# open-rmf/rmf_crowdsim

Hardware: AMD Instinct MI355X
Metric: agent-steps/sec at 1M agents, dt=0.05 s; % HBM roofline on Zanlungo kernel (higher is better)
Workload: dtype f32

## Files before the change

### include/crowdstep.h

```cpp
#ifndef CROWDSTEP_H
#define CROWDSTEP_H

#include <stddef.h>
#include <stdint.h>

#ifdef __cplusplus
extern "C" {
#endif

#define CS_ABI_VERSION 1

typedef struct cs_engine cs_engine;

typedef struct cs_grid_desc {
  double width;
  double height;
  double cell_size;
  double offset_x;
  double offset_y;
} cs_grid_desc;

typedef struct cs_device_cfg {
  int32_t device_ordinal;
  uint32_t flags;
// ... 112 lines not shown

uint32_t cs_abi_version(void);
cs_engine* cs_create(const cs_grid_desc* grid, const cs_device_cfg* cfg);
void cs_destroy(cs_engine*);
const char* cs_last_error(const cs_engine*);
const char* cs_backend_name(const cs_engine*);

uint32_t cs_register_zanlungo(cs_engine*, const cs_zanlungo_params*);
uint32_t cs_register_no_local_plan(cs_engine*);
uint32_t cs_register_lp_callback(cs_engine*, cs_lp_batch_fn fn, void* user);
uint32_t cs_register_hlp(cs_engine*, const cs_hlp_desc*);

int cs_add_agents(cs_engine*, const double* xy, size_t n, uint32_t hlp,
                  uint32_t lp, double eyesight, uint64_t* out_ids);
int cs_remove_agent(cs_engine*, uint64_t id);
uint32_t cs_add_source_sink(cs_engine*, const cs_source_sink_desc*);
void cs_remove_source_sink(cs_engine*, uint32_t handle);
size_t cs_source_sink_slots(cs_engine*);

int cs_step(cs_engine*, double dt_seconds, cs_step_report* report);
int cs_synchronize(cs_engine*);

size_t cs_agent_count(cs_engine*);
size_t cs_read_agents(cs_engine*, cs_agent_view* out, size_t cap);
size_t cs_drain_events(cs_engine*, cs_event* out, size_t cap);
void cs_event_recording(cs_engine*, int on);
typedef struct cs_snapshot_record {
  double x, y;
  float vx, vy;
  uint32_t id;
  uint32_t next_waypoint;
} cs_snapshot_record;
int cs_snapshot_request(cs_engine*);
int cs_snapshot_acquire(cs_engine*, int wait, const cs_snapshot_record** out,
                        size_t* n, uint64_t* step_index);
size_t cs_query_radius(cs_engine*, double radius, double x, double y,
                       uint64_t* out_ids, size_t cap);
size_t cs_query_knn(cs_engine*, size_t k, double x, double y, uint64_t* out_ids);

int cs_query_radius_batch(cs_engine*, size_t n, const double* xy, const double* radius, size_t cap_per_query,
                          uint64_t* out_ids, uint64_t* out_counts, float* out_d2, uint32_t* out_cells);
int cs_query_knn_batch(cs_engine*, size_t n, const double* xy, size_t k, uint64_t* out_ids, uint64_t* out_counts,
                       float* out_d2);

uint64_t cs_device_bytes(cs_engine*);

#define CS_STAT_WINDOWS_OFF_LDS 0u
#define CS_STAT_WINDOWS_CHUNKED 1u
#define CS_STAT_EXCHANGES_AHEAD 2u
#define CS_STAT_EXCHANGES_AHEAD_USED 3u
#define CS_STAT_STEPS_ON_KEPT_WINDOWS 4u
#define CS_STAT_RENUMBERINGS 5u
#define CS_STAT_RENUMBER_NS 6u
uint64_t cs_kernel_stat(cs_engine*, uint32_t which);

enum {
  CS_K_NEIGHBOUR_FORCE = 0,
  CS_K_SCAN = 1,
  CS_K_SCATTER = 2,
  CS_K_SPAWN = 3,
  CS_K_HALO = 4,
  CS_K_HALO_PACK = 5,
  CS_K_HALO_EXCHANGE = 6,
  CS_K_HALO_UNPACK = 7,
  CS_K_STEP_BORDER = 8,
  CS_K_STEP_INTERIOR = 9,
  CS_K_COUNT = 10
};
void cs_profile_enable(cs_engine*, uint32_t kernel_mask);
void cs_profile_stride(cs_engine*, uint32_t every);
int cs_profile_read(cs_engine*, uint32_t kernel, double* total_ms, uint64_t* launches);
void cs_profile_reset(cs_engine*);

enum { CS_DIR_XLO = 0, CS_DIR_XHI = 1, CS_DIR_YLO = 2, CS_DIR_YHI = 3,
       CS_DIR_XLO_YLO = 4, CS_DIR_XLO_YHI = 5, CS_DIR_XHI_YLO = 6, CS_DIR_XHI_YHI = 7 };
#define CS_HALO_RECORD_BYTES 40u
int cs_halo_set_buffers(cs_engine*, uint32_t dir, void* send_dev, void* recv_dev,
                        uint64_t capacity_records);
int cs_halo_pack(cs_engine*, uint32_t axis);
int cs_halo_unpack(cs_engine*, uint32_t axis);
int cs_halo_pack_all(cs_engine*);
int cs_halo_unpack_all(cs_engine*);
size_t cs_spawn_probe(cs_engine*, double dt_seconds, uint8_t* flags, size_t cap);
int cs_spawn_commit(cs_engine*, const uint8_t* flags, size_t n);
int cs_spawn_probe_dev(cs_engine*, double dt_seconds, int* flags_dev, size_t cap);
int cs_spawn_commit_dev(cs_engine*, const int* flags_dev, size_t n);

int cs_tile_histogram(cs_engine*, uint64_t* rows, uint64_t* cols);
size_t cs_tile_export(cs_engine*, void* records, size_t cap_records);
int cs_tile_retile(cs_engine*, uint32_t tile_cx0, uint32_t tile_cx1, uint32_t tile_cy0, uint32_t tile_cy1);
int cs_tile_import(cs_engine*, const void* records, size_t n);

typedef struct cs_route_miss {
  uint64_t id;
  uint32_t hlp;
  uint32_t slot;
  double px, py;
  double tx, ty;
} cs_route_miss;
size_t cs_route_misses(cs_engine*, cs_route_miss* out, size_t cap);
int cs_route_resolve(cs_engine*, const cs_route_miss* all, size_t n);

#define CS_RCCL_UNIQUE_ID_BYTES 128
int cs_rccl_unique_id(uint8_t* out_id);
int cs_rccl_comm_init(cs_engine*, int32_t n_ranks, int32_t rank, const uint8_t* id);
int cs_rccl_comm_adopt(cs_engine*, void* nccl_comm);
// ... 64 lines not shown
```

### rmf_crowdsim_amd/_abi.py

```python
import ctypes as C

CS_ABI_VERSION = 1

CS_CFG_DEFAULT = 0
CS_CFG_FORCE_GATHER = 1
CS_CFG_FORCE_TILED = 2
CS_CFG_DENSE = 4
CS_CFG_TILE_OVERLAP = 8
CS_CFG_WIDE_IDS = 16
CS_STAT_WINDOWS_OFF_LDS = 0
CS_STAT_WINDOWS_CHUNKED = 1
CS_STAT_EXCHANGES_AHEAD = 2
CS_STAT_EXCHANGES_AHEAD_USED = 3
CS_STAT_STEPS_ON_KEPT_WINDOWS = 4
CS_STAT_RENUMBERINGS = 5
CS_STAT_RENUMBER_NS = 6

CS_HLP_NONE, CS_HLP_CONSTANT, CS_HLP_ID_PARITY, CS_HLP_CALLBACK, CS_HLP_ROUTE = 0, 1, 2, 3, 4
CS_ROUTE_MAX_WAYPOINTS = 1023
CS_GEN_MONOTONIC, CS_GEN_POISSON_SEEDED, CS_GEN_CALLBACK = 0, 1, 2
CS_EVENT_SPAWNED, CS_EVENT_DESTROYED = 1, 2
(CS_K_NEIGHBOUR_FORCE, CS_K_SCAN, CS_K_SCATTER, CS_K_SPAWN, CS_K_HALO, CS_K_HALO_PACK, CS_K_HALO_EXCHANGE,
 CS_K_HALO_UNPACK, CS_K_STEP_BORDER, CS_K_STEP_INTERIOR, CS_K_COUNT) = range(11)
KERNEL_NAMES = ["neighbour_force", "scan", "scatter", "spawn", "halo", "halo_pack", "halo_exchange", "halo_unpack",
                "step_border", "step_interior"]
CS_DIR_XLO, CS_DIR_XHI, CS_DIR_YLO, CS_DIR_YHI = 0, 1, 2, 3
CS_DIR_XLO_YLO, CS_DIR_XLO_YHI, CS_DIR_XHI_YLO, CS_DIR_XHI_YHI = 4, 5, 6, 7
CS_HALO_RECORD_BYTES = 40
CS_RCCL_UNIQUE_ID_BYTES = 128
NO_SOURCE_SINK = 0xFFFFFFFF


class GridDesc(C.Structure):
    _fields_ = [("width", C.c_double), ("height", C.c_double), ("cell_size", C.c_double),
                ("offset_x", C.c_double), ("offset_y", C.c_double)]


class DeviceCfg(C.Structure):
    _fields_ = [("device_ordinal", C.c_int32), ("flags", C.c_uint32),
                ("tile_cx0", C.c_uint32), ("tile_cx1", C.c_uint32),
                ("tile_cy0", C.c_uint32), ("tile_cy1", C.c_uint32),
                ("halo_cells", C.c_uint32), ("reserved", C.c_uint32),
                ("capacity_hint", C.c_uint64), ("stream", C.c_void_p)]


class ZanlungoParams(C.Structure):
    _fields_ = [("agent_scale", C.c_double), ("obstacle_scale", C.c_double),
                ("reaction_time", C.c_double), ("force_distance", C.c_double),
                ("agent_mass", C.c_double), ("agent_radius", C.c_double)]


HlpVelocityFn = C.CFUNCTYPE(None, C.c_void_p, C.c_size_t, C.POINTER(C.c_uint64),
                            C.POINTER(C.c_double), C.POINTER(C.c_double), C.c_double,
                            C.POINTER(C.c_double), C.POINTER(C.c_uint8))
HlpSetTargetFn = C.CFUNCTYPE(None, C.c_void_p, C.c_uint64, C.c_double, C.c_double, C.c_double,
                             C.c_double, C.c_double, C.c_double)
HlpRemoveFn = C.CFUNCTYPE(None, C.c_void_p, C.c_uint64)
GeneratorFn = C.CFUNCTYPE(C.c_size_t, C.c_void_p, C.c_double)


class LpAgent(C.Structure):
    _fields_ = [("agent_id", C.c_uint64), ("x", C.c_double), ("y", C.c_double), ("vx", C.c_double),
                ("vy", C.c_double), ("preferred_vx", C.c_double), ("preferred_vy", C.c_double),
                ("eyesight_range", C.c_double), ("next_waypoint", C.c_uint64)]


LpBatchFn = C.CFUNCTYPE(C.c_int, C.c_void_p, C.c_size_t, C.POINTER(LpAgent), C.POINTER(C.c_double),
                        C.POINTER(C.c_uint64), C.POINTER(LpAgent), C.POINTER(C.c_double))

# ... 242 lines not shown
```

### rmf_crowdsim_amd/csrc/crowdstep_hip.hip

```cpp

#include <hip/hip_runtime.h>
#include <chrono>

#include <algorithm>
#include <cmath>
#include <cstdint>
#include <cstdio>
#include <array>
#include <cmath>
#include <cstring>
#include <map>
#include <string>
#include <thread>
#include <tuple>
#include <vector>

#include "crowdstep.h"
#include "crowdstep_state.h"

#define CS_INVALID_CELL 0xFFFFFFFFu
#define CS_MAX_GROUPS 1048575u
#define CS_SPAWN_OCCUPANCY_RADIUS 0.4
#define CS_ID_LIMIT 0x7FFFFFFFull

// ... 246 lines not shown
      ev.x = ev.y = 0;
      if (e->record_events) e->events.push_back(ev);
      return 0;
    }
  if (int rc = e->refresh_counts()) return rc;
  uint32_t found[2] = {0xFFFFFFFFu, 0u};
  uint64_t dev = 0;
  if (e->dev_id(id, &dev) && dev < 0xFFFFFFFFull && e->n_slots) {
    if (!e->find_dev && hipMalloc(&e->find_dev, 2 * sizeof(uint32_t)) != hipSuccess) {
      e->error = "HIP error while removing an agent";
      return 90;
    }
    bool ok = hipMemcpyAsync(e->find_dev, found, sizeof found, hipMemcpyHostToDevice, e->stream) == hipSuccess;
    hipLaunchKernelGGL(k_remove_by_id, dim3((e->n_slots + 255u) / 256u), dim3(256), 0, e->stream, e->buf[e->cur],
                       e->n_slots, e->ctr, e->gdev.tile, (uint32_t)dev, e->find_dev);
    ok = ok && hipMemcpyAsync(found, e->find_dev, sizeof found, hipMemcpyDeviceToHost, e->stream) == hipSuccess &&
         hipStreamSynchronize(e->stream) == hipSuccess;
    if (!ok) {
      e->error = "HIP error while removing an agent";
      return 90;
    }
  }
  if (found[0] == 0xFFFFFFFFu) {
    e->error = "unknown agent id";
    return 2;
  }
  const HostGroup& g = e->groups[meta_group(e->gdev, found[1])];
  const cs_hlp_desc& p = e->hlps[g.hlp];
  if (p.kind == CS_HLP_CALLBACK && p.remove_agent) p.remove_agent(p.user, id);
  e->sorted = false;
  e->hist_valid = false;
  e->occ_valid = false;
  e->halo_invalidate();
  e->n_alive_host -= 1;
  cs_event ev;
  ev.kind = CS_EVENT_DESTROYED;
  ev.source_sink = g.sink >= 0 ? (uint32_t)g.sink : UINT32_MAX;
  ev.id = id;
  ev.x = ev.y = 0;
  if (e->record_events) e->events.push_back(ev);
  return 0;
}

size_t cs_source_sink_slots(cs_engine* e) { return e->sinks.size(); }
uint64_t cs_device_bytes(cs_engine* e) { return e->device_bytes(); }

uint64_t cs_kernel_stat(cs_engine* e, uint32_t which) {
  hipSetDevice(e->device);
  if (which == CS_STAT_EXCHANGES_AHEAD) return e->n_exchanges_ahead;
  if (which == CS_STAT_EXCHANGES_AHEAD_USED) return e->n_exchanges_ahead_used;
  if (which == CS_STAT_STEPS_ON_KEPT_WINDOWS) return e->n_steps_on_kept_windows;
  if (which == CS_STAT_RENUMBERINGS) return e->n_renumberings;
  if (which == CS_STAT_RENUMBER_NS) return e->renumber_ns;
  Counters c;
  if (e->read_counters(&c)) return 0;
  switch (which) {
    case CS_STAT_WINDOWS_OFF_LDS: return c.n_win_off_lds;
    case CS_STAT_WINDOWS_CHUNKED: return c.n_win_chunked;
#ifdef CS_TILE_TRIPS
    case 100: case 101: case 102: case 103: case 104: case 105: case 106: case 107: case 108: case 109: case 110: case 111:
    case 112: case 113: case 114: case 115: case 116:
      return c.dbg[which - 100];
#endif
    default: return 0;
  }
}

uint32_t cs_add_source_sink(cs_engine* e, const cs_source_sink_desc* d) {
  if (d->n_waypoints == 0) {
    e->error = "a source-sink needs at least one waypoint";
    return UINT32_MAX;
  }
  hipSetDevice(e->device);
  if (e->room_for_group(d->n_waypoints)) return UINT32_MAX;
  HostSink s;
  s.d = *d;
  s.waypoints.assign(d->waypoints_xy, d->waypoints_xy + 2 * d->n_waypoints);
  s.d.waypoints_xy = nullptr;
  uint32_t handle = (uint32_t)e->sinks.size();
  if (e->tile && d->hlp < e->hlps.size() && e->hlps[d->hlp].kind == CS_HLP_ROUTE) {
    s.spawn_route = e->route_lookup(d->hlp, d->source_x, d->source_y, s.waypoints[0], s.waypoints[1]);
    if (!s.spawn_route) {
      e->error = "route planner found no route for this source-sink (tile engines plan at registration)";
      return UINT32_MAX;
    }
  }
  s.group = e->make_group(d->hlp, d->lp, d->agent_eyesight_range, (int32_t)handle);
  e->sinks.push_back(s);
  e->sinks_dirty = true;
  return handle;
}

void cs_remove_source_sink(cs_engine* e, uint32_t handle) {
  if (handle < e->sinks.size() && e->sinks[handle].alive) {
    e->sinks[handle].alive = false;
    e->sinks_dirty = true;
  }
}

int cs_step(cs_engine* e, double dt_seconds, cs_step_report* report) {
  hipSetDevice(e->device);
  const int rc = e->step(dt_seconds, report);
  if (rc == 0) e->steps_done += 1;
  return rc;
}

// ... 760 lines not shown
```

### rmf_crowdsim_amd/csrc/cs_engine.hip.inc

```

namespace {

inline uint64_t sat_usize(double v) {
  if (!(v > 0.0)) return 0;
  if (v >= 18446744073709551615.0) return UINT64_MAX;
  return (uint64_t)v;
}

inline uint64_t splitmix64(uint64_t x) {
  x += 0x9E3779B97F4A7C15ull;
  x = (x ^ (x >> 30)) * 0xBF58476D1CE4E5B9ull;
  x = (x ^ (x >> 27)) * 0x94D049BB133111EBull;
  return x ^ (x >> 31);
}
inline uint64_t poisson_seeded(uint64_t seed, uint64_t step, double mean) {
  if (!(mean > 0.0)) return 0;
  double limit = std::exp(-mean), prod = 1.0;
  uint64_t k = 0;
  for (uint64_t draw = 0; draw < 1000000; ++draw) {
    uint64_t r = splitmix64(seed ^ splitmix64(step * 0x100000001B3ull + draw));
    double u = (double)((r >> 11) + 1) * (1.0 / 9007199254740993.0);
    prod *= u;
    if (prod <= limit) break;
    ++k;
// ... 728 lines not shown
    if (hist_valid) return 0;
    HIP_OK(hipMemsetAsync(cell_count, 0, (ncells + 1) * sizeof(uint32_t), stream));
    if (n_slots)
      hipLaunchKernelGGL(k_count, dim3((n_slots + 255) / 256), dim3(256), 0, stream, buf[cur], 0u,
                         n_slots, cell_count, ctr, gdev.tile);
    HIP_OK(hipGetLastError());
    hist_valid = true;
    return 0;
  }

  uint32_t tile_agents_cap(int h) const {
    const uint32_t rb = tile_rows;
    if (rb <= 1)
      return std::min<uint32_t>(TILE_AGENTS_MAX, ((uint32_t)(2 * h + 1) * TILE_THREADS * 9u / 8u + 192u + tile_agents_slack + 63u) & ~63u);
    const double per_cell = (double)n_slots / (double)std::max<uint64_t>(ncells, 1);
    const double halo_cols = 2.0 * h * per_cell * 1.25;
    const double want = (rb + 2.0 * h) * ((double)tile_target / rb * 9.0 / 8.0 + halo_cols) + 64.0 + tile_agents_slack;
    const uint32_t base = ((rb + 2u * h) * (tile_target / rb) * 9u / 8u + 192u + tile_agents_slack + 63u) & ~63u;
    const uint32_t cap = std::max(base, ((uint32_t)want + 63u) & ~63u);
    return std::min<uint32_t>(TILE_AGENTS_MAX, cap);
  }

  bool bands_built = false;
  bool windows_shadow = true;
  uint32_t windows_keep_max_agents = 300000, windows_slack_pct = 10;
  bool windows_valid = false;
  bool scan_onepass = true;
  unsigned long long* scan_tile_sums = nullptr;
  uint32_t scan_seq = 0;
  uint32_t debug_sort_every = 0, debug_sort_phase = 0, debug_sorted_slots = 0;
  bool debug_sorted_once = false;
  bool debug_ctx_by_value = false;
  uint32_t scan_ticket_base = 0;
  uint32_t kept_agents_cap = 0;
  uint32_t windows_bound = 0;
  BlockDesc* blk_desc_back = nullptr;
  uint32_t* n_blocks_back = nullptr;
  struct WindowsKey {
    uint32_t ncells, nx, own_x0, own_x1, own_y0, own_y1, org_x, org_y, h, desc_cap, rows, target, stage_cap, split;
    const void* desc;
    bool operator==(const WindowsKey& o) const { return std::memcmp(this, &o, sizeof *this) == 0; }
  } windows_key{};
  int alloc_window_arrays(uint32_t cap_each) {
    hipFree(blk_desc);
    hipFree(blk_desc_back);
    blk_desc = blk_desc_back = nullptr;
    blk_desc_cap = cap_each;
    HIP_OK(hipMalloc(&blk_desc, (uint64_t)blk_desc_cap * sizeof(BlockDesc)));
    HIP_OK(hipMalloc(&blk_desc_back, (uint64_t)blk_desc_cap * sizeof(BlockDesc)));
    windows_valid = false;
    return 0;
  }
  uint64_t n_steps_on_kept_windows = 0;
  bool check_windows = false;
  std::string check_windows_error;
  int check_window_list(const BlockDesc* list_dev, const uint32_t* count_dev, uint32_t rows, uint32_t n_bands, uint32_t max_cols,
                        bool cover, uint32_t launch_windows) {
    HIP_OK(hipStreamSynchronize(stream));
    uint32_t cnt[2] = {0, 0};
    HIP_OK(hipMemcpy(cnt, count_dev, sizeof cnt, hipMemcpyDeviceToHost));
    char msg[512];
    if (cnt[0] > blk_desc_cap || cnt[0] > launch_windows) {
      std::snprintf(msg, sizeof msg, "window check: %u windows listed, the array holds %u, the launch %u", cnt[0], blk_desc_cap, launch_windows);
      check_windows_error = msg;
      error = check_windows_error.c_str();
      return 7;
    }
    std::vector<BlockDesc> d(cnt[0]);
    if (cnt[0]) HIP_OK(hipMemcpy(d.data(), list_dev, (size_t)cnt[0] * sizeof(BlockDesc), hipMemcpyDeviceToHost));
    const uint32_t ncols = gdev.own_y1 - gdev.own_y0;
    std::vector<std::vector<uint8_t>> seen(n_bands, std::vector<uint8_t>(cover ? ncols : 0u, 0));
    for (uint32_t k = 0; k < cnt[0]; ++k) {
      const BlockDesc& w = d[k];
      const bool in_rows = w.row0 >= gdev.own_x0 && w.row0 < gdev.own_x1 && (w.row0 - gdev.own_x0) % rows == 0u && w.nrows >= 1u &&
                           w.nrows <= rows && w.row0 + w.nrows <= gdev.own_x1;
      const bool in_cols = w.y0 <= w.y1 && w.y0 >= gdev.own_y0 && w.y1 < gdev.own_y1 &&
                           (w.y1 - w.y0 + 1u <= max_cols || ncols > BAND_LDS_COLS);
      if (!in_rows || !in_cols || w.count != 0u) {
        std::snprintf(msg, sizeof msg, "window check: window %u of %u is {row0 %u nrows %u y0 %u y1 %u first %u count %u}; owned rows [%u, %u) columns [%u, %u), %u rows per band, %u columns at most",
                      k, cnt[0], w.row0, w.nrows, w.y0, w.y1, w.first, w.count, gdev.own_x0, gdev.own_x1, gdev.own_y0, gdev.own_y1, rows, max_cols);
        check_windows_error = msg;
        error = check_windows_error.c_str();
        return 7;
      }
      if (cover) {
        std::vector<uint8_t>& band = seen[(w.row0 - gdev.own_x0) / rows];
        for (uint32_t y = w.y0; y <= w.y1; ++y) band[y - gdev.own_y0] += 1;
      }
    }
    if (cover)
      for (uint32_t b = 0; b < n_bands; ++b)
        for (uint32_t y = 0; y < ncols; ++y)
          if (seen[b][y] != 1) {
            std::snprintf(msg, sizeof msg, "window check: column %u of band %u is covered %u times (%u windows)", y, b, (unsigned)seen[b][y], cnt[0]);
            check_windows_error = msg;
            error = check_windows_error.c_str();
            return 7;
          }
    return 0;
  }
  uint32_t tile_max_cols(uint32_t h) const {
    const long long half = (long long)FIX_LIM / std::max(gdev.cs_fix, 1) - 2;
    const long long cols = 2 * half - 2 * (long long)h - 2;
    return (uint32_t)std::max<long long>(1, std::min<long long>(cols, 4096));
  }
  uint32_t split_margin() const {
    const bool wanted = ((flags & CS_CFG_TILE_OVERLAP) && rccl_comm != nullptr) || tile_split_force;
    return (tile && wanted && tile_rows > 1) ? halo_cells + 1u : 0u;
  }
  int rebuild(uint32_t bands = 0, uint32_t band_rows = 0, uint32_t band_h = 0, uint32_t band_stage_cap = 0,
              bool keep_windows = false, bool cover = false, uint32_t band_target = 0) {
    const bool bands_were_built = bands_built;
    bands_built = false;
    if (sorted) return 0;
    if (int rc = recount()) return rc;
    if (debug_sort_every > 1 && !tile && n_live_sinks == 0 && debug_sorted_once && !keep_windows && n_slots == debug_sorted_slots &&
        (++debug_sort_phase % debug_sort_every) != 0) {
      HIP_OK(hipMemsetAsync(cell_count, 0, (size_t)ncells * sizeof(uint32_t), stream));
      HIP_OK(hipMemsetAsync(&ctr->n_destroyed, 0, 6 * sizeof(uint32_t), stream));
      bands_built = bands_were_built;
      sorted = true;
      hist_valid = false;
      return 0;
    }
    debug_sorted_once = true;
    debug_sorted_slots = n_slots;
    prof_begin(CS_K_SCAN);
    uint32_t* const scan_clears = (keep_windows || windows_valid) ? n_blocks_back : n_blocks_dev;
    if (scan_onepass && n_scan_blocks <= SCAN_ONEPASS_MAX_BLOCKS) {
      if (!scan_tile_sums) {
        HIP_OK(hipMalloc(&scan_tile_sums, ((size_t)SCAN_ONEPASS_MAX_BLOCKS + 1) * sizeof(unsigned long long)));
        HIP_OK(hipMemsetAsync(scan_tile_sums, 0, ((size_t)SCAN_ONEPASS_MAX_BLOCKS + 1) * sizeof(unsigned long long), stream));
        scan_ticket_base = 0;
      }
      if (++scan_seq == 0u) scan_seq = 1u;
      hipLaunchKernelGGL(k_scan_onepass, dim3(n_scan_blocks), dim3(SCAN_BLOCK), 0, stream, cell_count, (uint32_t)ncells,
                         cell_start, ctr, scan_clears, scan_tile_sums, scan_seq,
                         reinterpret_cast<uint32_t*>(scan_tile_sums + SCAN_ONEPASS_MAX_BLOCKS), scan_ticket_base);
      scan_ticket_base += n_scan_blocks;
    } else {
// ... 1000 lines not shown
        if (++early_seq == 0u) early_seq = 1u;
        c2.flag_seq = early_seq;
        StepParams Pc = P;
        Pc.halo_late_check = fuse_pack ? 1u : 0u;
        {
          const dim3 grid(grid_blocks), block(TILE_THREADS);
          const EpilogueCore& Ec = static_cast<const EpilogueCore&>(E);
          if (ctx_by_value)
            hipLaunchKernelGGL((k_step_tiled<true, false, true>), grid, block, lds, stream, Pc, view(cur), Ep, Ec, cell_start, pref, blk_desc, n_blocks_dev, c2);
          else
            hipLaunchKernelGGL((k_step_tiled<false, false, true>), grid, block, lds, stream, Pc, view(cur), Ep, Ec, cell_start, pref, blk_desc, n_blocks_dev, c2);
        }
        border_on_aux = true;
        early_pending = true;
      } else if (n_slots && split) {
        TileCfg cfg_b = cfg;
        cfg_b.part = 1;
        cfg_b.spill = tile_spill + (uint64_t)grid_blocks * cfg.spill_rows * TILE_THREADS;
        hipStream_t sb = stream;
        border_on_aux = false;
        if (overlap_ready && (!need_host || fire_and_forget)) {
          if (int rc = ensure_aux()) return rc;
          HIP_OK(hipEventRecord(ev_sorted, stream));
          HIP_OK(hipStreamWaitEvent(aux_stream, ev_sorted, 0));
          sb = aux_stream;
          border_on_aux = true;
        }
        const int tb = prof_open_on(CS_K_STEP_BORDER, sb);
        launch_tiled(sb, P, cfg_b);
        prof_close_on(tb, sb);
        if (border_on_aux) HIP_OK(hipEventRecord(ev_border, aux_stream));
        StepParams Pi = P;
        Pi.halo_late_check = fuse_pack ? 1u : 0u;
        const int ti = prof_open_on(CS_K_STEP_INTERIOR, stream);
        launch_tiled(stream, Pi, cfg);
        prof_close_on(ti, stream);
        if (border_on_aux) HIP_OK(hipStreamWaitEvent(stream, ev_border, 0));
      } else if (n_slots) {
        launch_tiled(stream, P, cfg);
      }
      prof_end();
    } else {
      if (tile)
        hipLaunchKernelGGL(k_build_blocks, dim3(1), dim3(1024), 0, stream, gdev, cell_start, blk_desc,
                           blk_desc_cap, n_blocks_dev, ctr);
      if (n_slots && P.peek_seq) flight_launched(P.peek_seq);
      prof_begin(CS_K_NEIGHBOUR_FORCE);
      if (n_slots)
        hipLaunchKernelGGL(k_step_gather, dim3((n_slots + 255) / 256), dim3(256), 0, stream, P, view(cur),
                           Ep, cell_start, pref);
      prof_end();
    }
    HIP_OK(hipGetLastError());
    if (builders && check_windows)
      if (int rc = check_window_list(blk_desc_back, n_blocks_back, tile_rows, n_bands, tile_max_cols((uint32_t)h), true, 0xFFFFFFFFu)) return rc;
    if (builders) {
      std::swap(blk_desc, blk_desc_back);
      std::swap(n_blocks_dev, n_blocks_back);
    }
    windows_valid = want_keep && n_slots != 0u && tiled && (builders != 0u || (keep_now && had_windows) || (!keep_now && bands_built) || cover_built_late);
    if (windows_valid && (builders != 0u || !keep_now)) windows_bound = band_windows_max;
    if (windows_valid) kept_agents_cap = agents_cap_now;
    if (fuse_pack) {
      halo_prepacked = true;
      halo_all_clean = false;
      halo_counts_clean[0] = halo_counts_clean[1] = false;
    }

    if (!need_host || fire_and_forget) {
      cur ^= 1;
      sorted = false;
      hist_valid = true;
      occ_valid = has_sinks;
      if (has_sinks || tile) {
        counts_stale = true;
        ++async_steps;
      }
      errors_stale = true;
      spawn_committed = false;
      committed_spawns = 0;
      slots_added = 0;
      ghosts_present = false;
      return 0;
    }

    Counters c;
    if (int rc = read_counters(&c)) return rc;
    counts_stale = false;
    errors_stale = false;
    async_steps = 0;
    if (has_sinks && (!tile || spawn_on_device)) next_id = c.next_id;
    const uint64_t first_spawn_id = (uint64_t)c.next_id - c.n_spawned;
    if (c.n_scan_stalled) {
      poisoned = true;
      error = poison_error = kScanStalled;
      return 7;
    }
    if (c.n_out_of_bounds || limbo_fail) {
      HIP_OK(hipMemsetAsync(&ctr->n_out_of_bounds, 0, sizeof(uint32_t), stream));
      HIP_OK(hipMemsetAsync(cell_count, 0, (ncells + 1) * sizeof(uint32_t), stream));
      hist_valid = false;
      occ_valid = false;
      halo_invalidate();
      n_alive_host = c.n_alive;
      n_slots = c.n_alive;
      if (!spawn_events_done) finish_spawn_events(c.n_spawned, first_spawn_id);
// ... 436 lines not shown
```

### rmf_crowdsim_amd/csrc/cs_kernel_band_builder.hip.inc

```
  __shared__ uint32_t wsum[4];
  __shared__ uint32_t s_carry;
  const int lane = threadIdx.x & 63, wave = threadIdx.x >> 6;
  const uint32_t row0 = g.own_x0 + band * rb;
  const uint32_t nown = min(rb, g.own_x1 - row0);
  const uint32_t ncols = g.own_y1 - g.own_y0;
  BAND_ARRAY(uint32_t, s_incl, BAND_LDS_COLS)
  uint32_t* __restrict__ incl =
      ncols <= BAND_LDS_COLS ? s_incl : prefix + (unsigned long long)band * ncols;
  auto column_count = [&](uint32_t y) {
    uint32_t c = 0;
    for (uint32_t r = 0; r < nown; ++r) {
      const unsigned long long q = (unsigned long long)(row0 + r) * g.nx + g.own_y0 + y;
      c += cell_start[q + 1] - cell_start[q];
    }
    return c;
  };
  if (threadIdx.x == 0) s_carry = 0;
  __syncthreads();
  BAND_ARRAY(uint32_t, s_all, BAND_LDS_COLS)
  const uint32_t hl = min(h, g.own_y0), hr = min(h, g.nx - g.own_y1);
  const uint32_t ncols_ext = ncols + hl + hr;
  const uint32_t gr0 = row0 > h ? row0 - h : 0u;
  const uint32_t gr1 = min(row0 + nown - 1u + h, g.ncells / g.nx - 1u);
  const bool staged_prefix = ncols_ext <= BAND_LDS_COLS;
// ... 60 lines not shown
    uint32_t run = w - mine, run_a = wa - mine_a;
    for (int k = 0; k < wave; ++k) {
      run += wsum[k];
      run_a += wsum_a[k];
    }
#pragma unroll
    for (uint32_t k = 0; k < EPT; ++k) {
      const uint32_t y = threadIdx.x * EPT + k;
      run += c[k];
      run_a += ca[k];
      if (y < ncols) s_incl[y] = run;
      if (staged_prefix && y < ncols_ext) s_all[y] = run_a;
    }
    if (threadIdx.x == blockDim.x - 1) s_carry = run;
    __syncthreads();
  } else {
    for (uint32_t base = 0; base < ncols; base += blockDim.x) {
      const uint32_t y = base + threadIdx.x;
      const uint32_t c = y < ncols ? column_count(y) : 0u;
      const uint32_t w = wave_incl_scan(c, lane);
      if (lane == 63) wsum[wave] = w;
      __syncthreads();
      uint32_t woff = 0;
      for (int k = 0; k < wave; ++k) woff += wsum[k];
      if (y < ncols) incl[y] = s_carry + woff + w;
      __syncthreads();
      if (threadIdx.x == blockDim.x - 1) s_carry += woff + w;
      __syncthreads();
    }
  }
  const uint32_t total = s_carry;
  if (threadIdx.x == 0) {
    if (total) atomicAdd(&ctr->n_owned, total);
  }
  auto lb = [&](uint32_t v) {
    uint32_t lo = 0, hi = ncols;
    while (lo < hi) {
      const uint32_t mid = (lo + hi) >> 1;
      if (incl[mid] >= v) hi = mid; else lo = mid + 1;
    }
    return lo;
  };
  const bool band_border = split && (row0 < g.own_x0 + split || row0 + nown + split > g.own_x1);
  auto is_border = [&](uint32_t y0, uint32_t y1) {
    return split && (band_border || y0 < split || y1 + split >= ncols);
  };
  const uint32_t list_cap = split ? desc_cap / 2u : desc_cap;
  auto emit = [&](uint32_t k, bool border, uint32_t y0, uint32_t y1) {
    if (k >= list_cap) atomicAdd(&ctr->n_win_dropped, 1u);
    if (k < list_cap) {
      k = border ? desc_cap - 1u - k : k;
      BlockDesc d;
      d.row0 = row0;
      d.nrows = nown;
      d.y0 = g.own_y0 + y0;
      d.y1 = g.own_y0 + y1;
      d.first = 0;
      d.count = 0;
      desc[k] = d;
    }
  };
  if (ncols <= BAND_LDS_COLS) {
    BAND_ARRAY(unsigned short, s_end, BAND_LDS_COLS)
    BAND_ARRAY(unsigned short, s_next, BAND_LDS_COLS)
    BAND_ARRAY(unsigned short, s_win, BAND_LDS_COLS)
    BAND_ARRAY(unsigned short, s_cls, BAND_LDS_COLS)
    __shared__ uint32_t s_nw, s_first, s_first_b, s_y0;
    if (threadIdx.x == 0) s_y0 = ncols;
    __syncthreads();
    constexpr int NQ = 4;
    int halvings = 1;
    while ((1u << halvings) <= ncols_ext) ++halvings;
    auto lb_many = [&](const uint32_t (&v)[2 * NQ], uint32_t (&out)[2 * NQ], auto staged_tag) {
      constexpr bool STAGED = decltype(staged_tag)::value;
      uint32_t lo[2 * NQ], hi[2 * NQ];
#pragma unroll
      for (int k = 0; k < 2 * NQ; ++k) {
        lo[k] = 0;
        hi[k] = (STAGED && k >= NQ) ? ncols_ext : ncols;
      }
      for (int it = 0; it < halvings; ++it) {
        uint32_t mid[2 * NQ], x[2 * NQ];
#pragma unroll
        for (int k = 0; k < 2 * NQ; ++k) {
          mid[k] = (lo[k] + hi[k]) >> 1;
          if (STAGED && k >= NQ) x[k] = s_all[min(mid[k], ncols_ext - 1u)];
          else x[k] = s_incl[min(mid[k], ncols - 1u)];
        }
#pragma unroll
        for (int k = 0; k < 2 * NQ; ++k) {
          const bool open = lo[k] < hi[k], ge = x[k] >= v[k];
          hi[k] = (open && ge) ? mid[k] : hi[k];
          lo[k] = (open && !ge) ? mid[k] + 1u : lo[k];
        }
      }
#pragma unroll
      for (int k = 0; k < 2 * NQ; ++k) out[k] = lo[k];
    };
    const uint32_t own_share = (uint32_t)(((unsigned long long)stage_cap * nown) / (nown + 2u * h));
    for (uint32_t base = 0; base < ncols; base += NQ * blockDim.x) {
      uint32_t y[NQ], e_prev[NQ], vab[2 * NQ], yab[2 * NQ];
      bool live[NQ];
#pragma unroll
      for (int k = 0; k < NQ; ++k) {
        y[k] = base + k * blockDim.x + threadIdx.x;
        const uint32_t yy = min(y[k], ncols - 1u);
        e_prev[k] = yy == 0 ? 0u : s_incl[yy - 1];
        live[k] = y[k] < ncols && s_incl[yy] != e_prev[k];
        vab[k] = e_prev[k] + target + 1u;
        if (staged_prefix) {
          const uint32_t yl = yy + hl > h ? yy + hl - h : 0u;
          vab[NQ + k] = (yl == 0u ? 0u : s_all[yl - 1u]) + stage_cap + 1u;
        } else {
          const uint32_t yl = yy > h ? yy - h : 0u;
          vab[NQ + k] = (yl == 0u ? 0u : s_incl[yl - 1u]) + own_share + 1u;
        }
      }
      if (staged_prefix) lb_many(vab, yab, std::true_type{});
      else lb_many(vab, yab, std::false_type{});
      uint32_t y1[NQ], vcd[2 * NQ], ycd[2 * NQ];
// ... 103 lines not shown
```

### rmf_crowdsim_amd/csrc/cs_kernels_step.hip.inc

```

struct WpEvent {
  uint32_t id, group, next_wp, cell;
  float ox, oy;
  uint32_t slot, pad;
};

struct EpilogueCore {
  AgentArrays out;
  uint32_t* cell_count;
  Counters* ctr;
  const GroupDev* groups;
  const SinkDev* sinks;
  const double* waypoints;
  double grid_off_x, grid_off_y, cell_size;
  uint2* destroyed;
  uint32_t destroyed_cap;
  WpEvent* wp_events;
  uint32_t wp_events_cap;
  const uint32_t* src_cell_start;
  const uint32_t* src_sorted;
  uint32_t* src_occupied;
  const uint2* route_desc;
  const double* route_xy;
  const RouteBookEntry* route_book;
// ... 297 lines not shown
  if (i >= E.ctr->n_alive) {
    E.out.cell[i] = CS_INVALID_CELL;
    return;
  }
  if (E.ctr->n_out_of_bounds != 0u) return;
  const uint32_t cell = in.cell[i];
  Own o;
  o.gx = cell / P.g.nx;
  o.gy = cell - o.gx * P.g.nx;
  if (P.g.tile && (o.gx < P.g.own_x0 || o.gx >= P.g.own_x1 || o.gy < P.g.own_y0 || o.gy >= P.g.own_y1)) {
    E.out.cell[i] = CS_INVALID_CELL;
    return;
  }
  o.off = in.off[i];
  o.v = in.vel[i];
  o.id = in.id[i];
  o.slot = i;
  const uint32_t meta = in.meta[i];
  const GroupDev grp = E.groups[meta_group(P.g, meta)];
  uint32_t route_st = in.route ? in.route[i] : 0u;
  o.u = hlp_velocity(grp, E, P.g, o.id, pref, i, o.gx, o.gy, o.off, route_st);
  float wx = o.u.x, wy = o.u.y;
  if (grp.lp_kind == 2u && E.lp_vel) {
    wx = E.lp_vel[i].x;
    wy = E.lp_vel[i].y;
  }
  if (grp.lp_kind == 1u && o.off.x == o.off.x && o.off.y == o.off.y) {
    bool tz;
    gather_agent(P, in, cell_start, o, grp, wx, wy, tz);
    if (tz) atomicAdd(&E.ctr->n_tti_zero, 1u);
  }
  step_epilogue(P, E, Ep, i, o.gx, o.gy, o.off, o.id, meta, grp, wx, wy, route_st, P.halo_late_check);
}

__global__ void __launch_bounds__(256) k_lp_recommended(StepParams P, AgentArrays in, const EpilogueCtx* __restrict__ Ep,
                                                        const float2* __restrict__ pref, float2* __restrict__ out) {
  const EpilogueCtx& E = *Ep;
  const uint32_t i = blockIdx.x * blockDim.x + threadIdx.x;
  if (i >= P.n || i >= E.ctr->n_alive) return;
  const uint32_t cell = in.cell[i];
  const uint32_t meta = in.meta[i];
  const GroupDev grp = E.groups[meta_group(P.g, meta)];
  if (grp.lp_kind != 2u) return;
  const uint32_t gx = cell / P.g.nx, gy = cell - gx * P.g.nx;
  uint32_t route_st = in.route ? in.route[i] : 0u;
  out[i] = hlp_velocity(grp, E, P.g, in.id[i], pref, i, gx, gy, in.off[i], route_st);
}

#ifndef TILE_THREADS
#define TILE_THREADS 256
#endif

struct BlockDesc {
  uint32_t row0, nrows, y0, y1, first, count;
};

__global__ void __launch_bounds__(1024) k_build_blocks(GridDev g, const uint32_t* __restrict__ cell_start,
                                                       BlockDesc* __restrict__ desc, uint32_t desc_cap,
                                                       uint32_t* __restrict__ n_blocks,
                                                       Counters* __restrict__ ctr) {
  __shared__ uint32_t wsum[16];
  __shared__ uint32_t s_carry, s_owned;
  if (threadIdx.x == 0) {
    s_carry = 0;
    s_owned = 0;
  }
  __syncthreads();
  const int lane = threadIdx.x & 63, wave = threadIdx.x >> 6;
  const uint32_t n_rows = g.own_x1 - g.own_x0;
  for (uint32_t base = 0; base < n_rows; base += blockDim.x) {
    uint32_t R = g.own_x0 + base + threadIdx.x;
    uint32_t first = 0, cnt = 0;
    if (R < g.own_x1) {
      first = cell_start[(unsigned long long)R * g.nx + g.own_y0];
      cnt = cell_start[(unsigned long long)R * g.nx + g.own_y1] - first;
    }
    uint32_t nb = (cnt + TILE_THREADS - 1u) / TILE_THREADS;
    uint32_t incl = wave_incl_scan(nb, lane);
    if (lane == 63) wsum[wave] = incl;
    if (cnt) atomicAdd(&s_owned, cnt);
    __syncthreads();
    uint32_t woff = 0;
    for (int w = 0; w < wave; ++w) woff += wsum[w];
    uint32_t excl = s_carry + woff + incl - nb;
    for (uint32_t k = 0; k < nb; ++k) {
      if (excl + k < desc_cap) {
        BlockDesc d;
        d.row0 = R;
        d.nrows = 1;
        d.y0 = d.y1 = 0;
        d.first = first + k * TILE_THREADS;
        d.count = min((uint32_t)TILE_THREADS, cnt - k * TILE_THREADS);
        desc[excl + k] = d;
      }
    }
    __syncthreads();
    if (threadIdx.x == blockDim.x - 1) s_carry = excl + nb;
    __syncthreads();
  }
  if (threadIdx.x == 0) {
    *n_blocks = min(s_carry, desc_cap);
    ctr->n_owned = s_owned;
    ctr->n_pending = cell_start[g.ncells];
  }
}

#define BAND_LDS_COLS 2048
__device__ __forceinline__ void build_band(const uint32_t band, const GridDev& g,
                                           const uint32_t* __restrict__ cell_start, uint32_t rb,
                                           uint32_t target, uint32_t h, uint32_t stage_cap,
                                           uint32_t max_cols, uint32_t split, uint32_t cover, uint32_t* __restrict__ prefix,
                                           BlockDesc* __restrict__ desc, uint32_t desc_cap,
                                           uint32_t* __restrict__ n_blocks, Counters* __restrict__ ctr) {
#define BAND_ARRAY(type, name, count) __shared__ type name[count];
#include "cs_kernel_band_builder.hip.inc"
#undef BAND_ARRAY
}

#define BAND_OFF_s_incl 0u
#define BAND_OFF_s_all (BAND_LDS_COLS * 4u)
#define BAND_OFF_s_end (BAND_LDS_COLS * 8u)
#define BAND_OFF_s_next (BAND_LDS_COLS * 10u)
#define BAND_OFF_s_win (BAND_LDS_COLS * 12u)
#define BAND_OFF_s_cls (BAND_LDS_COLS * 14u)
#define BAND_SCRATCH_BYTES (BAND_LDS_COLS * 16u)
__device__ __noinline__ void build_band_in(unsigned char* band_scratch, const uint32_t band, const GridDev& g,
                                           const uint32_t* __restrict__ cell_start, uint32_t rb,
                                           uint32_t target, uint32_t h, uint32_t stage_cap,
                                           uint32_t max_cols, uint32_t split, uint32_t cover, uint32_t* __restrict__ prefix,
                                           BlockDesc* __restrict__ desc, uint32_t desc_cap,
                                           uint32_t* __restrict__ n_blocks, Counters* __restrict__ ctr) {
#define BAND_ARRAY(type, name, count) type* const name = reinterpret_cast<type*>(band_scratch + BAND_OFF_##name);
#include "cs_kernel_band_builder.hip.inc"
#undef BAND_ARRAY
}


__global__ void __launch_bounds__(256) k_build_bands(GridDev g, const uint32_t* __restrict__ cell_start,
                                                     uint32_t rb, uint32_t target, uint32_t h,
                                                     uint32_t stage_cap, uint32_t max_cols, uint32_t split, uint32_t cover,
                                                     uint32_t* __restrict__ prefix,
                                                     BlockDesc* __restrict__ desc, uint32_t desc_cap,
// ... 138 lines not shown
  if (EARLY && cfg.split == 2u) {
    n_first = min(n_blocks[1], cfg.desc_cap >> 1);
    part = lidx < n_first ? 1u : 0u;
    widx = part ? lidx : lidx - n_first;
    if (lidx == 0 && threadIdx.x == 0 && n_first + min(n_blocks[0], cfg.desc_cap >> 1) > gridDim.x - n_builders)
      atomicAdd(&E.ctr->n_win_dropped, 1u);
    if (lidx == 0 && threadIdx.x == 0 && n_first == 0u)
      __hip_atomic_store(&E.ctr->border_flag, cfg.flag_seq, __ATOMIC_RELEASE, __HIP_MEMORY_SCOPE_AGENT);
  }
  if (!(EARLY && cfg.split == 2u) && widx == 0 && threadIdx.x == 0 && n_blocks[part] > min(gridDim.x - n_builders, cfg.desc_cap >> (cfg.split ? 1 : 0)))
    atomicAdd(&E.ctr->n_win_dropped, 1u);
  if (widx >= min(n_blocks[part], cfg.desc_cap >> (cfg.split ? 1 : 0))) return;
  const uint32_t late_check = (EARLY && cfg.split == 2u && part) ? 0u : P.halo_late_check;
#define BORDER_DONE()                                                                                              \
  do {                                                                                                             \
    if (EARLY && cfg.split == 2u && part) {                                                                        \
      __syncthreads();                                                                                             \
      if (threadIdx.x == 0) {                                                                                      \
        __threadfence();                                                                                           \
        if (atomicAdd(&E.ctr->border_done, 1u) + 1u == n_first) {                                                  \
          E.ctr->border_done = 0u;                                                                                 \
          __hip_atomic_store(&E.ctr->border_flag, cfg.flag_seq, __ATOMIC_RELEASE, __HIP_MEMORY_SCOPE_AGENT);      \
        }                                                                                                          \
      }                                                                                                            \
    }                                                                                                              \
  } while (0)
  PHASE_BEGIN();
  __builtin_amdgcn_s_setprio(3);
  const BlockDesc d = desc[part ? cfg.desc_cap - 1u - widx : widx];
#ifdef CS_PHASE_CLOCKS
  if (d.row0 == 0xFFFFFFF0u) return;
#endif
  PHASE_MARK(0);
  const GridDev g = P.g;
  const int tid = threadIdx.x;
  int2* __restrict__ s_pos = reinterpret_cast<int2*>(smem);
  float2* __restrict__ s_vel = reinterpret_cast<float2*>(s_pos + cfg.agents_cap);
  uint32_t* __restrict__ s_id = reinterpret_cast<uint32_t*>(s_vel + cfg.agents_cap);
  entry_t* __restrict__ s_list = reinterpret_cast<entry_t*>(s_id + cfg.agents_cap);
  uint32_t* __restrict__ s_idtmp = reinterpret_cast<uint32_t*>(s_list);
  unsigned short* __restrict__ s_tab =
      reinterpret_cast<unsigned short*>(s_list + (cfg.list_cap + TILE_LIST_SPARE) * TILE_THREADS);

  __shared__ uint32_t s_rfirst[TILE_MAX_OWN_ROWS], s_rpref[TILE_MAX_OWN_ROWS + 1];
  __shared__ unsigned short s_self[TILE_THREADS];
  __shared__ uint32_t s_huge;
  __shared__ uint32_t s_dead;
  if (threadIdx.x == 0) {
    s_huge = 0u;
    s_dead = E.ctr->n_out_of_bounds;
  }
  const int n_rows = (int)(g.ncells / g.nx);
  const int row0 = (int)d.row0, nown = (int)d.nrows;
  const bool strip = d.count != 0;
  int ylo, yhi;
  if (strip) {
    const uint32_t c_lo = in.cell[d.first], c_hi = in.cell[d.first + d.count - 1];
    ylo = (int)(c_lo - (uint32_t)row0 * g.nx);
    yhi = (int)(c_hi - (uint32_t)row0 * g.nx);
  } else {
    ylo = (int)d.y0;
    yhi = (int)d.y1;
  }
  const int sy0 = max(ylo - cfg.h, 0), sy1 = min(yhi + cfg.h, (int)g.nx - 1);
  const int W1 = sy1 - sy0 + 2;
  const int r0 = max(row0 - cfg.h, 0), r1 = min(row0 + nown - 1 + cfg.h, n_rows - 1);
  const int nr = r1 - r0 + 1;
  if (tid < nr) {
    unsigned long long rowbase = (unsigned long long)(r0 + tid) * g.nx;
    uint32_t g0 = cell_start[rowbase + sy0], g1 = cell_start[rowbase + sy1 + 1];
    s_g0[tid] = g0;
    s_rc[tid + 1] = g1 - g0;
  }
  if (tid >= 64 && tid < 64 + nown) {
    const int r = tid - 64;
    if (strip) {
      s_rfirst[0] = d.first;
      s_rpref[1] = d.count;
    } else {
      const unsigned long long rowbase = (unsigned long long)(row0 + r) * g.nx;
      const uint32_t f = cell_start[rowbase + ylo];
      s_rfirst[r] = f;
      s_rpref[r + 1] = cell_start[rowbase + yhi + 1] - f;
    }
  }
  __syncthreads();
  if (s_dead != 0u) {
    BORDER_DONE();
    return;
  }
  if (tid == 0) {
    uint32_t acc = 0, pad = 0;
    s_rc[0] = 0;
    s_base[0] = 0;
    for (int k = 0; k < nr; ++k) {
      const uint32_t c = s_rc[k + 1];
      acc += c;
      pad += (c + 2u) & ~1u;
      s_rc[k + 1] = acc;
      s_base[k + 1] = pad;
    }
    acc = 0;
    s_rpref[0] = 0;
    for (int k = 0; k < nown; ++k) {
      uint32_t c = s_rpref[k + 1];
      s_rpref[k + 1] = acc + c;
      acc += c;
    }
  }
  __syncthreads();
  const uint32_t S_real = s_rc[nr];
  const uint32_t S = s_base[nr];
  const uint32_t n_own = s_rpref[nown];
  if constexpr (WITH_BUILDERS) {
    if (n_own == 0u) {
      BORDER_DONE();
      return;
    }
  }
  const int kc = nr / 2, cyc = W1 / 2;
  const bool tiled_ok = S + 2u <= cfg.agents_cap && S < 65533u && (uint32_t)(nr * W1) <= cfg.table_cap &&
                        (long long)(W1 / 2 + 2) * g.cs_fix <= (long long)FIX_LIM &&
                        (long long)(nr / 2 + 2) * g.cs_fix <= (long long)FIX_LIM;

  struct OwnIn {
    uint32_t i, cell, id, meta, route;
    float2 off, v;
    GroupDev grp;
    int own_r;
    bool active;
  };
// ... 729 lines not shown
```

### rust/rmf_crowdsim_gpu/src/ffi.rs

```rust

#![allow(non_camel_case_types)]

use std::os::raw::{c_char, c_int, c_void};

pub const CS_ABI_VERSION: u32 = 1;

pub const CS_CFG_DEFAULT: u32 = 0;
pub const CS_CFG_FORCE_GATHER: u32 = 1;
pub const CS_CFG_FORCE_TILED: u32 = 2;
pub const CS_CFG_DENSE: u32 = 4;
pub const CS_CFG_TILE_OVERLAP: u32 = 8;
pub const CS_CFG_WIDE_IDS: u32 = 16;
pub const CS_STAT_WINDOWS_OFF_LDS: u32 = 0;
pub const CS_STAT_WINDOWS_CHUNKED: u32 = 1;
pub const CS_STAT_EXCHANGES_AHEAD: u32 = 2;
pub const CS_STAT_EXCHANGES_AHEAD_USED: u32 = 3;
pub const CS_STAT_STEPS_ON_KEPT_WINDOWS: u32 = 4;
pub const CS_STAT_RENUMBERINGS: u32 = 5;
pub const CS_STAT_RENUMBER_NS: u32 = 6;

pub const CS_HLP_NONE: u32 = 0;
pub const CS_HLP_CONSTANT: u32 = 1;
pub const CS_HLP_ID_PARITY: u32 = 2;
pub const CS_HLP_CALLBACK: u32 = 3;
pub const CS_HLP_ROUTE: u32 = 4;
pub const CS_ROUTE_MAX_WAYPOINTS: usize = 1023;

pub const CS_GEN_MONOTONIC: u32 = 0;
pub const CS_GEN_POISSON_SEEDED: u32 = 1;
pub const CS_GEN_CALLBACK: u32 = 2;

pub const CS_EVENT_SPAWNED: u32 = 1;
pub const CS_EVENT_DESTROYED: u32 = 2;

pub const CS_K_NEIGHBOUR_FORCE: u32 = 0;
pub const CS_K_SCAN: u32 = 1;
pub const CS_K_SCATTER: u32 = 2;
pub const CS_K_SPAWN: u32 = 3;
pub const CS_K_HALO: u32 = 4;
pub const CS_K_HALO_PACK: u32 = 5;
pub const CS_K_HALO_EXCHANGE: u32 = 6;
pub const CS_K_HALO_UNPACK: u32 = 7;
pub const CS_K_STEP_BORDER: u32 = 8;
pub const CS_K_STEP_INTERIOR: u32 = 9;
pub const CS_K_COUNT: u32 = 10;

pub const CS_DIR_XLO: u32 = 0;
pub const CS_DIR_XHI: u32 = 1;
pub const CS_DIR_YLO: u32 = 2;
pub const CS_DIR_YHI: u32 = 3;
pub const CS_DIR_XLO_YLO: u32 = 4;
pub const CS_DIR_XLO_YHI: u32 = 5;
pub const CS_DIR_XHI_YLO: u32 = 6;
pub const CS_DIR_XHI_YHI: u32 = 7;
pub const CS_HALO_RECORD_BYTES: u32 = 40;
pub const CS_RCCL_UNIQUE_ID_BYTES: usize = 128;

#[repr(C)]
pub struct cs_engine {
    _private: [u8; 0],
}

#[repr(C)]
pub struct cs_mesh {
    _private: [u8; 0],
}

pub type cs_mesh_exchange_fn = Option<unsafe extern "C" fn(user: *mut c_void, n: usize, peers: *const i32, send_tags: *const i32, recv_tags: *const i32, send_host: *const *const c_void, recv_host: *const *mut c_void, bytes: *const usize) -> c_int>;
pub type cs_mesh_allreduce_max_fn = Option<unsafe extern "C" fn(user: *mut c_void, values: *mut i32, n: usize) -> c_int>;
pub type cs_mesh_allgather_fn = Option<unsafe extern "C" fn(user: *mut c_void, mine: *const c_void, bytes: usize, all: *mut c_void) -> c_int>;
#[repr(C)]
#[derive(Clone, Copy)]
// ... 258 lines not shown
```

Before: 6.931 billion.

## Cut band windows at exact agent-count boundaries for balanced tiles

Adds a path in the band builder that splits each band of one or two rows into windows holding a fixed target number of agents. Each window records exact per-row slot ranges (first/count, first1/count1), and the step kernel reads them instead of deriving ranges from cell boundaries. The aim is to balance work across tiled blocks and avoid underfilled or oversized windows. In exchange the descriptor grows from 24 to 32 bytes, builder logic becomes more complex, and the window checker and a listed-windows stat are extended.

```diff
diff --git a/include/crowdstep.h b/include/crowdstep.h
--- a/include/crowdstep.h
+++ b/include/crowdstep.h
@@ -188,6 +188,7 @@
 #define CS_STAT_STEPS_ON_KEPT_WINDOWS 4u
 #define CS_STAT_RENUMBERINGS 5u
 #define CS_STAT_RENUMBER_NS 6u
+#define CS_STAT_WINDOWS_LISTED 7u
 uint64_t cs_kernel_stat(cs_engine*, uint32_t which);
 
 enum {
diff --git a/rmf_crowdsim_amd/_abi.py b/rmf_crowdsim_amd/_abi.py
--- a/rmf_crowdsim_amd/_abi.py
+++ b/rmf_crowdsim_amd/_abi.py
@@ -15,6 +15,7 @@
 CS_STAT_STEPS_ON_KEPT_WINDOWS = 4
 CS_STAT_RENUMBERINGS = 5
 CS_STAT_RENUMBER_NS = 6
+CS_STAT_WINDOWS_LISTED = 7
 
 CS_HLP_NONE, CS_HLP_CONSTANT, CS_HLP_ID_PARITY, CS_HLP_CALLBACK, CS_HLP_ROUTE = 0, 1, 2, 3, 4
 CS_ROUTE_MAX_WAYPOINTS = 1023
diff --git a/rmf_crowdsim_amd/csrc/crowdstep_hip.hip b/rmf_crowdsim_amd/csrc/crowdstep_hip.hip
--- a/rmf_crowdsim_amd/csrc/crowdstep_hip.hip
+++ b/rmf_crowdsim_amd/csrc/crowdstep_hip.hip
@@ -322,6 +322,10 @@
   if (which == CS_STAT_STEPS_ON_KEPT_WINDOWS) return e->n_steps_on_kept_windows;
   if (which == CS_STAT_RENUMBERINGS) return e->n_renumberings;
   if (which == CS_STAT_RENUMBER_NS) return e->renumber_ns;
+  if (which == CS_STAT_WINDOWS_LISTED) {
+    uint64_t n = 0;
+    return e->windows_listed(&n) ? 0 : n;
+  }
   Counters c;
   if (e->read_counters(&c)) return 0;
   switch (which) {
diff --git a/rmf_crowdsim_amd/csrc/cs_engine.hip.inc b/rmf_crowdsim_amd/csrc/cs_engine.hip.inc
--- a/rmf_crowdsim_amd/csrc/cs_engine.hip.inc
+++ b/rmf_crowdsim_amd/csrc/cs_engine.hip.inc
@@ -804,6 +804,16 @@
     return 0;
   }
   uint64_t n_steps_on_kept_windows = 0;
+  const uint32_t* last_windows_count = nullptr;
+  int windows_listed(uint64_t* out) {
+    *out = 0;
+    if (!last_windows_count) return 0;
+    uint32_t cnt[2] = {0, 0};
+    HIP_OK(hipStreamSynchronize(stream));
+    HIP_OK(hipMemcpy(cnt, last_windows_count, sizeof cnt, hipMemcpyDeviceToHost));
+    *out = (uint64_t)cnt[0] + cnt[1];
+    return 0;
+  }
   bool check_windows = false;
   std::string check_windows_error;
   int check_window_list(const BlockDesc* list_dev, const uint32_t* count_dev, uint32_t rows, uint32_t n_bands, uint32_t max_cols,
@@ -822,22 +832,64 @@
     if (cnt[0]) HIP_OK(hipMemcpy(d.data(), list_dev, (size_t)cnt[0] * sizeof(BlockDesc), hipMemcpyDeviceToHost));
     const uint32_t ncols = gdev.own_y1 - gdev.own_y0;
     std::vector<std::vector<uint8_t>> seen(n_bands, std::vector<uint8_t>(cover ? ncols : 0u, 0));
+    std::vector<uint32_t> cs((size_t)ncells + 1u);
+    HIP_OK(hipMemcpy(cs.data(), cell_start, ((size_t)ncells + 1u) * sizeof(uint32_t), hipMemcpyDeviceToHost));
+    const uint32_t own_rows = gdev.own_x1 - gdev.own_x0;
+    std::vector<std::vector<std::pair<uint32_t, uint32_t>>> runs(own_rows);
     for (uint32_t k = 0; k < cnt[0]; ++k) {
       const BlockDesc& w = d[k];
       const bool in_rows = w.row0 >= gdev.own_x0 && w.row0 < gdev.own_x1 && (w.row0 - gdev.own_x0) % rows == 0u && w.nrows >= 1u &&
                            w.nrows <= rows && w.row0 + w.nrows <= gdev.own_x1;
       const bool in_cols = w.y0 <= w.y1 && w.y0 >= gdev.own_y0 && w.y1 < gdev.own_y1 &&
                            (w.y1 - w.y0 + 1u <= max_cols || ncols > BAND_LDS_COLS);
-      if (!in_rows || !in_cols || w.count != 0u) {
-        std::snprintf(msg, sizeof msg, "window check: window %u of %u is {row0 %u nrows %u y0 %u y1 %u first %u count %u}; owned rows [%u, %u) columns [%u, %u), %u rows per band, %u columns at most",
-                      k, cnt[0], w.row0, w.nrows, w.y0, w.y1, w.first, w.count, gdev.own_x0, gdev.own_x1, gdev.own_y0, gdev.own_y1, rows, max_cols);
+      bool cut_ok = w.cut ? (!cover && w.nrows <= 2u && w.count + w.count1 >= 1u && w.count + w.count1 <= (uint32_t)TILE_THREADS &&
+                             (w.nrows == 2u || w.count1 == 0u))
+                          : (w.count == 0u && w.count1 == 0u);
+      if (in_rows && in_cols && cut_ok && w.cut) {
+        bool at_y0 = false, at_y1 = false;
+        for (uint32_t r = 0; r < w.nrows; ++r) {
+          const uint32_t f = r ? w.first1 : w.first, c = r ? w.count1 : w.count;
+          if (!c) continue;
+          const size_t q = (size_t)(w.row0 + r) * gdev.nx;
+          cut_ok = cut_ok && f >= cs[q + w.y0] && f + c <= cs[q + w.y1 + 1u];
+          at_y0 = at_y0 || (f < cs[q + w.y0 + 1u]);
+          at_y1 = at_y1 || (f + c > cs[q + w.y1]);
+        }
+        cut_ok = cut_ok && at_y0 && at_y1;
+      }
+      if (!in_rows || !in_cols || !cut_ok) {
+        std::snprintf(msg, sizeof msg, "window check: window %u of %u is {row0 %u nrows %u cut %u y0 %u y1 %u first %u count %u first1 %u count1 %u}; owned rows [%u, %u) columns [%u, %u), %u rows per band, %u columns at most",
+                      k, cnt[0], w.row0, (unsigned)w.nrows, (unsigned)w.cut, w.y0, w.y1, w.first, w.count, w.first1, w.count1, gdev.own_x0, gdev.own_x1, gdev.own_y0, gdev.own_y1, rows, max_cols);
         check_windows_error = msg;
         error = check_windows_error.c_str();
         return 7;
       }
+      for (uint32_t r = 0; r < w.nrows; ++r) {
+        const size_t q = (size_t)(w.row0 + r) * gdev.nx;
+        const uint32_t f = w.cut ? (r ? w.first1 : w.first) : cs[q + w.y0];
+        const uint32_t c = w.cut ? (r ? w.count1 : w.count) : cs[q + w.y1 + 1u] - f;
+        if (c) runs[w.row0 + r - gdev.own_x0].push_back({f, f + c});
+      }
       if (cover) {
         std::vector<uint8_t>& band = seen[(w.row0 - gdev.own_x0) / rows];
         for (uint32_t y = w.y0; y <= w.y1; ++y) band[y - gdev.own_y0] += 1;
+      }
+    }
+    for (uint32_t r = 0; r < own_rows && ncols <= BAND_LDS_COLS; ++r) {
+      std::sort(runs[r].begin(), runs[r].end());
+      const size_t q = (size_t)(gdev.own_x0 + r) * gdev.nx;
+      uint32_t at = cs[q + gdev.own_y0], bad = 0xFFFFFFFFu;
+      for (const auto& s : runs[r]) {
+        if (s.first != at && bad == 0xFFFFFFFFu) bad = std::min(at, s.first);
+        at = s.second;
+      }
+      if (at != cs[q + gdev.own_y1] && bad == 0xFFFFFFFFu) bad = std::min(at, cs[q + gdev.own_y1]);
+      if (bad != 0xFFFFFFFFu) {
+        std::snprintf(msg, sizeof msg, "window check: the windows' slots of row %u do not tile its owned slots [%u, %u) exactly once (%zu runs, %u windows; first gap or overlap at slot %u)",
+                      gdev.own_x0 + r, cs[q + gdev.own_y0], cs[q + gdev.own_y1], runs[r].size(), cnt[0], bad);
+        check_windows_error = msg;
+        error = check_windows_error.c_str();
+        return 7;
       }
     }
     if (cover)
@@ -1944,6 +1996,7 @@
       prof_end();
     }
     HIP_OK(hipGetLastError());
+    last_windows_count = (tiled && n_slots) ? n_blocks_dev : nullptr;
     if (builders && check_windows)
       if (int rc = check_window_list(blk_desc_back, n_blocks_back, tile_rows, n_bands, tile_max_cols((uint32_t)h), true, 0xFFFFFFFFu)) return rc;
     if (builders) {
diff --git a/rmf_crowdsim_amd/csrc/cs_kernel_band_builder.hip.inc b/rmf_crowdsim_amd/csrc/cs_kernel_band_builder.hip.inc
--- a/rmf_crowdsim_amd/csrc/cs_kernel_band_builder.hip.inc
+++ b/rmf_crowdsim_amd/csrc/cs_kernel_band_builder.hip.inc
@@ -136,11 +136,14 @@
       k = border ? desc_cap - 1u - k : k;
       BlockDesc d;
       d.row0 = row0;
-      d.nrows = nown;
+      d.nrows = (unsigned short)nown;
+      d.cut = 0;
       d.y0 = g.own_y0 + y0;
       d.y1 = g.own_y0 + y1;
       d.first = 0;
       d.count = 0;
+      d.first1 = 0;
+      d.count1 = 0;
       desc[k] = d;
     }
   };
@@ -150,6 +153,78 @@
     BAND_ARRAY(unsigned short, s_win, BAND_LDS_COLS)
     BAND_ARRAY(unsigned short, s_cls, BAND_LDS_COLS)
     __shared__ uint32_t s_nw, s_first, s_first_b, s_y0;
+    const uint32_t n_cut = (total + target - 1u) / max(target, 1u);
+    if (!cover && nown <= 2u && staged_prefix && target != 0u && target <= (uint32_t)TILE_THREADS && total != 0u &&
+        n_cut <= BAND_LDS_COLS) {
+      __shared__ uint32_t s_cut_bad;
+      if (threadIdx.x == 0) s_cut_bad = 0u;
+      __syncthreads();
+      auto lb_lds = [&](uint32_t v) {
+        uint32_t lo = 0, hi = ncols;
+        while (lo < hi) {
+          const uint32_t mid = (lo + hi) >> 1;
+          if (s_incl[mid] >= v) hi = mid; else lo = mid + 1;
+        }
+        return lo;
+      };
+      for (uint32_t k = threadIdx.x; k < n_cut; k += blockDim.x) {
+        const uint32_t p0 = k * target, p1 = min(p0 + target, total);
+        const uint32_t ya = lb_lds(p0 + 1u), yb = lb_lds(p1);
+        const uint32_t yl = ya + hl > h ? ya + hl - h : 0u;
+        const uint32_t yr = min(yb + hl + h, ncols_ext - 1u);
+        const uint32_t staged = s_all[yr] - (yl == 0u ? 0u : s_all[yl - 1u]);
+        if (staged > stage_cap || yb - ya + 1u > max_cols) s_cut_bad = 1u;
+        s_win[k] = (unsigned short)ya;
+        s_end[k] = (unsigned short)yb;
+      }
+      __syncthreads();
+      if (s_cut_bad == 0u) {
+        if (threadIdx.x == 0) {
+          uint32_t nb = 0;
+          if (split)
+            for (uint32_t w = 0; w < n_cut; ++w) {
+              const bool b = is_border(s_win[w], s_end[w]);
+              s_cls[w] = (unsigned short)(b ? (nb | 0x8000u) : (w - nb));
+              nb += b ? 1u : 0u;
+            }
+          s_first = n_cut - nb ? atomicAdd(&n_blocks[0], n_cut - nb) : 0u;
+          s_first_b = nb ? atomicAdd(&n_blocks[1], nb) : 0u;
+        }
+        __syncthreads();
+        auto row_slot = [&](uint32_t r, uint32_t p, uint32_t y) {
+          const unsigned long long q = (unsigned long long)(row0 + r) * g.nx + g.own_y0 + y;
+          const uint32_t at = cell_start[q];
+          if (y >= ncols) return at;
+          const uint32_t in_col = p - (y == 0u ? 0u : s_incl[y - 1u]);
+          if (nown == 1u) return at + in_col;
+          const uint32_t c0 = cell_start[q - (unsigned long long)r * g.nx + 1u] - cell_start[q - (unsigned long long)r * g.nx];
+          return r == 0u ? at + min(in_col, c0) : at + (in_col > c0 ? in_col - c0 : 0u);
+        };
+        for (uint32_t k = threadIdx.x; k < n_cut; k += blockDim.x) {
+          const uint32_t p0 = k * target, p1 = min(p0 + target, total);
+          const uint32_t ya = s_win[k], yb = s_end[k];
+          const uint32_t ye = p1 < total ? lb_lds(p1 + 1u) : ncols;
+          const bool b = split && (s_cls[k] & 0x8000u) != 0u;
+          uint32_t idx = (b ? s_first_b : s_first) + (split ? (s_cls[k] & 0x7FFFu) : k);
+          if (idx >= list_cap) atomicAdd(&ctr->n_win_dropped, 1u);
+          if (idx < list_cap) {
+            idx = b ? desc_cap - 1u - idx : idx;
+            BlockDesc d;
+            d.row0 = row0;
+            d.nrows = (unsigned short)nown;
+            d.cut = 1;
+            d.y0 = g.own_y0 + ya;
+            d.y1 = g.own_y0 + yb;
+            d.first = row_slot(0u, p0, ya);
+            d.count = row_slot(0u, p1, ye) - d.first;
+            d.first1 = nown > 1u ? row_slot(1u, p0, ya) : 0u;
+            d.count1 = nown > 1u ? row_slot(1u, p1, ye) - d.first1 : 0u;
+            desc[idx] = d;
+          }
+        }
+        return;
+      }
+    }
     if (threadIdx.x == 0) s_y0 = ncols;
     __syncthreads();
     constexpr int NQ = 4;
diff --git a/rmf_crowdsim_amd/csrc/cs_kernels_step.hip.inc b/rmf_crowdsim_amd/csrc/cs_kernels_step.hip.inc
--- a/rmf_crowdsim_amd/csrc/cs_kernels_step.hip.inc
+++ b/rmf_crowdsim_amd/csrc/cs_kernels_step.hip.inc
@@ -373,8 +373,11 @@
 #endif
 
 struct BlockDesc {
-  uint32_t row0, nrows, y0, y1, first, count;
+  uint32_t row0;
+  unsigned short nrows, cut;
+  uint32_t y0, y1, first, count, first1, count1;
 };
+static_assert(sizeof(BlockDesc) == 32, "a descriptor is two 16-byte scalar loads");
 
 __global__ void __launch_bounds__(1024) k_build_blocks(GridDev g, const uint32_t* __restrict__ cell_start,
                                                        BlockDesc* __restrict__ desc, uint32_t desc_cap,
@@ -409,6 +412,8 @@
         BlockDesc d;
         d.row0 = R;
         d.nrows = 1;
+        d.cut = 0;
+        d.first1 = d.count1 = 0;
         d.y0 = d.y1 = 0;
         d.first = first + k * TILE_THREADS;
         d.count = min((uint32_t)TILE_THREADS, cnt - k * TILE_THREADS);
@@ -653,7 +658,7 @@
   }
   const int n_rows = (int)(g.ncells / g.nx);
   const int row0 = (int)d.row0, nown = (int)d.nrows;
-  const bool strip = d.count != 0;
+  const bool strip = d.count != 0 && !d.cut;
   int ylo, yhi;
   if (strip) {
     const uint32_t c_lo = in.cell[d.first], c_hi = in.cell[d.first + d.count - 1];
@@ -678,6 +683,9 @@
     if (strip) {
       s_rfirst[0] = d.first;
       s_rpref[1] = d.count;
+    } else if (d.cut) {
+      s_rfirst[r] = r ? d.first1 : d.first;
+      s_rpref[r + 1] = r ? d.count1 : d.count;
     } else {
       const unsigned long long rowbase = (unsigned long long)(row0 + r) * g.nx;
       const uint32_t f = cell_start[rowbase + ylo];
diff --git a/rust/rmf_crowdsim_gpu/src/ffi.rs b/rust/rmf_crowdsim_gpu/src/ffi.rs
--- a/rust/rmf_crowdsim_gpu/src/ffi.rs
+++ b/rust/rmf_crowdsim_gpu/src/ffi.rs
@@ -18,6 +18,7 @@
 pub const CS_STAT_STEPS_ON_KEPT_WINDOWS: u32 = 4;
 pub const CS_STAT_RENUMBERINGS: u32 = 5;
 pub const CS_STAT_RENUMBER_NS: u32 = 6;
+pub const CS_STAT_WINDOWS_LISTED: u32 = 7;
 
 pub const CS_HLP_NONE: u32 = 0;
 pub const CS_HLP_CONSTANT: u32 = 1;
```

Result: faster. 7.296 billion (median of 6 runs) (+5.3%).
